# ANSSI-FR/libecc

Measured on AMD Instinct MI355X. Metric: scalar-mults/sec (secp256r1, batch=2^20, variable base, affine out, bit-exact vs CPU), higher is better.
Workload: dtype u32 (29-bit limbs, v_mad_u64_u32 integer MAD, u64 accumulators)

## Files before the change

### libecc_amd/csrc/ecamd_host.cpp

```cpp
#include <hip/hip_runtime.h>
#include <stdint.h>
#include <string.h>
#include <strings.h>
#include <stdio.h>
#include <stdlib.h>
#include <string>
#include <vector>
#include <functional>
#include <mutex>
#include <sys/random.h>

#include "../../include/libecc_amd.h"
#include "ecamd_internal.h"

static thread_local std::string g_err;
static int fail(const std::string &m)
{
	g_err = m;
	return -1;
}
#define HIPCHK(expr) \
	do { \
		hipError_t e_ = (expr); \
		if (e_ != hipSuccess) { \
// ... 1205 lines not shown
				(void)hipFree(dd);
			}
			std::vector<uint32_t> tab4((size_t)65 * 8 * 40, 0);
			for (uint32_t e = 0; ok && e < ne; e++) {
				ok = hst[e] == 0;
				big_digits29(&tab4[(size_t)e * 40], 9, big_mulmod(big_from_be(&hp[(size_t)e * 64], 32), R261, cv->p));
				big_digits29(&tab4[(size_t)e * 40 + 9], 9, big_mulmod(big_from_be(&hp[(size_t)e * 64 + 32], 32), R261, cv->p));
			}
			if (ok && hipMalloc((void **)&cv->d_comb4, tab4.size() * 4) == hipSuccess &&
			    hipMemcpy(cv->d_comb4, tab4.data(), tab4.size() * 4, hipMemcpyHostToDevice) != hipSuccess) {
				(void)hipFree(cv->d_comb4);
				cv->d_comb4 = nullptr;
			}
			(void)hipGetLastError();
		}
	}
	*out = cv;
	return 0;
}

extern "C" int ecamd_curve_by_name(ecamd_ctx *ctx, const char *name, ecamd_curve **out)
{
	if (!ctx || !name || !out) {
		return fail("ecamd_curve_by_name: NULL argument");
	}
	*out = nullptr;
	for (const CurveRow &r : g_curve_rows) {
		if (strcasecmp(r.name, name) == 0) {
			ecamd_curve *cv = new ecamd_curve();
			cv->curve_type = r.type;
			cv->p = big_from_hex(r.p);
			cv->a = big_from_hex(r.a);
			cv->b = big_from_hex(r.b);
			cv->order = big_from_hex(r.order);
			cv->gx = big_from_hex(r.gx);
			cv->gy = big_from_hex(r.gy);
			cv->q = big_from_hex(r.q);
			return curve_finish(ctx, cv, out);
		}
	}
	return fail(std::string("ecamd_curve_by_name: unknown curve ") + name);
}

extern "C" int ecamd_curve_from_params(ecamd_ctx *ctx, const uint8_t *p, uint32_t p_len, const uint8_t *a,
				       uint32_t a_len, const uint8_t *b, uint32_t b_len,
				       const uint8_t *curve_order, uint32_t curve_order_len,
				       const uint8_t *gx, uint32_t gx_len, const uint8_t *gy, uint32_t gy_len,
				       const uint8_t *gen_order, uint32_t gen_order_len, ecamd_curve **out)
{
	if (!ctx || !p || !a || !b || !curve_order || !gx || !gy || !gen_order || !out) {
		return fail("ecamd_curve_from_params: NULL argument");
	}
	*out = nullptr;
	ecamd_curve *cv = new ecamd_curve();
	cv->p = big_from_be(p, p_len);
	cv->a = big_from_be(a, a_len);
	cv->b = big_from_be(b, b_len);
	cv->order = big_from_be(curve_order, curve_order_len);
	cv->gx = big_from_be(gx, gx_len);
	cv->gy = big_from_be(gy, gy_len);
	cv->q = big_from_be(gen_order, gen_order_len);
	return curve_finish(ctx, cv, out);
}

extern "C" void ecamd_curve_free(ecamd_curve *cv)
{
	if (!cv) {
		return;
	}
	{
		std::lock_guard<std::mutex> lk(cv->ctx->mu);
		(void)hipSetDevice(cv->ctx->device);
		(void)hipStreamSynchronize(cv->ctx->stream);
		curve_free_device(cv);
	}
	curve_release_slots(cv);
	delete cv;
}

extern "C" int ecamd_curve_coord_len(const ecamd_curve *cv) { return cv ? cv->clen : -1; }
extern "C" int ecamd_curve_order_len(const ecamd_curve *cv) { return cv ? cv->qlen : -1; }
extern "C" int ecamd_curve_words(const ecamd_curve *cv) { return cv ? cv->nw : -1; }

#define P256_TAB_BYTES 512u
#define P256_SCRATCH_PER_ITEM ((size_t)P256_TAB_BYTES + 70u * 16u)

static size_t tbl_bytes_for(const ecamd_curve *cv, uint32_t stride)
{
	return (size_t)ECAMD_TBL_ENTRIES * 3 * (size_t)cv->nw * 4 * (size_t)stride;
}

static void maybe_build_comb(ecamd_ctx *ctx, ecamd_curve *cv, uint32_t n)
{
	if (cv->d_comb || cv->comb_off || ctx->comb_min_batch == 0 || n < ctx->comb_min_batch) {
		return;
	}
	const bool p256 = cv->is_p256;
	if (!p256 && cv->gslot < 0) {
		return;
	}
	cv->comb_off = true;
	if (hipDeviceSynchronize() != hipSuccess) {
		return;
	}
	const uint32_t nwords = (uint32_t)((cv->pbits + 31) / 32);
	const uint32_t slen = 4 * nwords, nwin = 2 * nwords;
	const uint32_t ne = nwin * 32768u + 1u;
	const uint32_t ew = p256 ? 20u : ecamd_g29_comb_entry_words(cv->pbits, cv->gflavour);
	if (!p256 && ne != ecamd_g29_comb_entries(cv->pbits)) {
		return;
	}
	std::vector<uint8_t> hs((size_t)ne * slen, 0);
	for (uint32_t j = 0; j < nwin; j++) {
		for (uint32_t m = 1; m <= 32768; m++) {
			uint8_t *e = &hs[((size_t)j * 32768 + (m - 1)) * slen];
			e[slen - 1 - 2 * j] = (uint8_t)(m & 0xff);
			e[slen - 2 - 2 * j] = (uint8_t)(m >> 8);
		}
	}
	big_to_be(&hs[(size_t)nwin * 32768 * slen], (int)slen, big_mod(big_pow2(8 * (int)slen), cv->q));
	const size_t plen = (size_t)2 * cv->clen;
	uint8_t *dsc = nullptr, *dpt = nullptr, *dst = nullptr;
	uint32_t *table = nullptr;
	std::vector<uint8_t> st(ne);
	hipStream_t s = ctx->stream;
	bool ok = hipMalloc((void **)&dsc, hs.size()) == hipSuccess && hipMalloc((void **)&dpt, (size_t)ne * plen) == hipSuccess &&
		  hipMalloc((void **)&dst, ne) == hipSuccess && hipMalloc((void **)&table, (size_t)ne * ew * 4) == hipSuccess &&
		  hipMemcpy(dsc, hs.data(), hs.size(), hipMemcpyHostToDevice) == hipSuccess;
	{
		const uint32_t user_chunk = ctx->max_chunk;
		ctx->max_chunk = user_chunk < (1u << 20) ? (1u << 20) : user_chunk;
		ok = ok && smul_dev_locked(ctx, cv, ne, dsc, slen, nullptr, dpt, dst, s) == 0;
		ctx->max_chunk = user_chunk;
	}
	if (ok) {
		const hipError_t e = p256 ? ecamd_launch_comb_build_p256(dpt, ne, table, s)
					  : ecamd_g29_comb_build(cv->pbits, cv->gslot, dpt, ne, (uint32_t)cv->clen, table, s, cv->gflavour);
		ok = e == hipSuccess && hipMemcpyAsync(st.data(), dst, ne, hipMemcpyDeviceToHost, s) == hipSuccess &&
		     hipStreamSynchronize(s) == hipSuccess;
	}
	for (uint32_t i = 0; ok && i < ne; i++) {
		ok = (st[i] == 0);
	}
	(void)hipFree(dsc);
	(void)hipFree(dpt);
	(void)hipFree(dst);
	if (!ok) {
		(void)hipFree(table);
		(void)hipGetLastError();
		return;
	}
	cv->d_comb = table;
	cv->comb_off = false;
}

static void maybe_build_comb4(ecamd_ctx *ctx, ecamd_curve *cv)
{
	static const bool off = getenv("ECAMD_NO_SECRET_COMB") != nullptr;
	if (off || cv->d_comb4 || cv->comb4_off || cv->is_p256 || cv->gslot < 0) {
		return;
	}
	cv->comb4_off = true;
	if (hipDeviceSynchronize() != hipSuccess) {
		return;
	}
	const uint32_t nwords = (uint32_t)((cv->pbits + 31) / 32);
	const uint32_t slen = 4 * nwords, nwin = 8 * nwords, ne = nwin * 8u + 1u;
	const uint32_t ew = ecamd_g29_comb_entry_words(cv->pbits, cv->gflavour);
// ... 4289 lines not shown
```

### libecc_amd/csrc/ecamd_internal.h

```cpp
#pragma once
#include <stdlib.h>
#include <hip/hip_runtime.h>
#include <stdint.h>

#define ECAMD_WINDOW 4
#define ECAMD_TBL_ENTRIES (1 << ECAMD_WINDOW)
#define ECAMD_STATUS_TAB 0xFC
#define ECAMD_STATUS_JAC 0xFD
#define ECAMD_STATUS_REDO 0xFE
#define ECAMD_MAX_SLOTS_HOST 16

struct EcamdSmulArgs {
	const uint8_t *scalars;
	const uint8_t *points;
	uint8_t *out;
	uint8_t *status;
	uint32_t *tbl;
	uint32_t *stg;
	uint32_t n, slen, clen, pstride, stride;
	uint32_t sstride;
	int slot;
	int only_redo;
	const uint32_t *lut;
	uint32_t lut_kind;
	int masked;
	const uint8_t *scalars2;
	uint32_t s2len;
};
#define ECAMD_COMB_ENTRIES (16u * 32768u + 1u)

struct EcamdFpArgs {
	const uint32_t *a, *b;
	uint32_t *out;
	uint32_t n, wstride;
	int op;
	int slot;
};

struct EcamdPtArgs {
	const uint8_t *p1, *p2;
	uint8_t *out, *status;
	uint32_t n, clen;
	int dbl, slot;
};

struct EcamdPtfArgs {
	const uint8_t *p1, *p2;
	uint8_t *out, *status;
	uint32_t n, clen;
	int op;
	int in_fmt, out_fmt, slot;
};
struct EcamdUnprotArgs {
	const uint8_t *points;
	const uint8_t *scalars;
	uint8_t *out, *status;
	uint32_t n, clen, slen, sstride;
	int in_fmt, out_fmt, slot;
};
hipError_t ecamd_launch_ptf(int nw, const EcamdPtfArgs &a, hipStream_t s);
hipError_t ecamd_launch_unprot(int nw, const EcamdUnprotArgs &a, hipStream_t s);

struct EcamdEcdsaPrepArgs {
	const uint8_t *sigs;
	const uint8_t *digests;
	uint8_t *u1, *u2;
	uint8_t *flags;
	uint32_t n, qlen, hlen, qbits;
	int qslot;
	const uint8_t *only;
};
struct EcamdEcdsaFinArgs {
	const uint8_t *A, *stA;
	const uint8_t *B, *stB;
	const uint8_t *sigs, *flags;
	uint8_t *result;
	uint32_t n, clen, qlen, jmax;
	uint32_t q[17];
	int slot;
	const uint8_t *only;
};
struct EcamdEcdsaSignArgs {
	const uint8_t *privs, *nonces, *digests;
	const uint8_t *kG, *stkG;
	uint8_t *sigs, *status;
	uint32_t n, clen, qlen, hlen, qbits, jmax;
	int qslot;
};
hipError_t ecamd_launch_ecdsa_sign(int nw, const EcamdEcdsaSignArgs &a, hipStream_t s);
hipError_t ecamd_launch_ecdsa_prep(int nw, const EcamdEcdsaPrepArgs &a, hipStream_t s);
hipError_t ecamd_launch_ecdsa_fin(int nw, const EcamdEcdsaFinArgs &a, hipStream_t s);

int ecamd_nw_supported(int nw);
// ... 435 lines not shown
```

### libecc_amd/csrc/ecamd_p256.h

```cpp
#pragma once
#include "ecamd_u29.h"

namespace p256 {
using namespace u29;

struct K {
	static constexpr u32 R2[9] = {0x00000c00, 0x00000000, 0x1fff0000, 0x1fdfffff, 0x1fbfffff,
				      0x1fffffff, 0x1fffffff, 0x1ffffffe, 0x00000013};
	static constexpr u32 ONE[9] = {0x00000020, 0x00000000, 0x00000000, 0x1fffc000, 0x1fffffff,
				       0x1fffffff, 0x1f7fffff, 0x03ffffff, 0x00000000};
	static constexpr u32 BM[9] = {0x1897bbfb, 0x1cdf6229, 0x018486c4, 0x01732821, 0x1dad59e0,
				      0x0abf7212, 0x1a06d110, 0x17721d20, 0x008600c3};
};

template <class T> U29_FN T constant(const u32 (&c)[9])
{
	T r;
#pragma unroll
	for (int i = 0; i < 9; i++) {
		r.l[i] = c[i];
	}
	return r;
}

// ... 57 lines not shown
	const auto t4 = sub<1, 1>(beta4, x3);
	const auto y3a = mul(alpha, t4);
	const auto y3 = carry(sub<2, 1>(y3a, g8));
	const auto z3 = mul_small<2>(mul(P.Y, P.Z));
	Jac R;
	R.X = weaken<FX>(x3);
	R.Y = weaken<FY>(y3);
	R.Z = weaken<FZ>(z3);
	return R;
}

template <class FX2, class FY2, class FZ2>
U29_FN Jac add_jac(const Jac &P, const FX2 &X2, const FY2 &Y2, const FZ2 &Z2, bool &h_is_zero)
{
	const auto z1z1 = sqr(P.Z);
	const auto z2z2 = sqr(Z2);
	const auto u1 = mul(P.X, z2z2);
	const auto u2 = mul(X2, z1z1);
	const auto s1 = mul(mul(P.Y, Z2), z2z2);
	const auto s2 = mul(mul(Y2, P.Z), z1z1);
	const auto h = carry(sub<1, 0>(u2, u1));
	const auto r = carry(sub<1, 0>(s2, s1));
	const auto hh = sqr(h);
	const auto hhh = mul(h, hh);
	const auto v = mul(u1, hh);
	const auto r2 = sqr(r);
	const auto x3 = fold(sub<2, 2>(r2, add(hhh, mul_small<2>(v))));
	const auto t5 = sub<1, 1>(v, x3);
	const auto m1 = mul(r, t5);
	const auto m2 = mul(s1, hhh);
	const auto y3 = carry(sub<1, 0>(m1, m2));
	const auto z3 = mul(mul(P.Z, Z2), h);
	h_is_zero = is_zero_mulout(z3);
	Jac R;
	R.X = weaken<FX>(x3);
	R.Y = weaken<FY>(y3);
	R.Z = weaken<FZ>(z3);
	return R;
}

typedef F<(1ull << 29) + MASK, (3ull << 24), 48> FYaff;
template <class FY2> U29_FN Jac madd(const Jac &P, const Fcanon &X2, const FY2 &Y2, bool &h_is_zero)
{
	const auto z1z1 = sqr(P.Z);
	const auto u2 = mul(X2, z1z1);
	const auto s2 = mul(mul(Y2, P.Z), z1z1);
	const auto h = carry(sub<1, 1>(u2, P.X));
	const auto r = carry(sub<3, 1>(s2, P.Y));
	const auto hh = sqr(h);
	const auto hhh = mul(h, hh);
	const auto v = mul(P.X, hh);
	const auto r2 = sqr(r);
	const auto x3 = fold(sub<2, 2>(r2, add(hhh, mul_small<2>(v))));
	const auto t5 = sub<1, 1>(v, x3);
	const auto y3 = carry(sub<1, 0>(mul(r, t5), mul(P.Y, hhh)));
	const auto z3 = mul(P.Z, h);
	h_is_zero = is_zero_mulout(z3);
	Jac R;
	R.X = weaken<FX>(x3);
	R.Y = weaken<FY>(y3);
	R.Z = weaken<FZ>(z3);
	return R;
}
U29_FN FYaff neg_aff(const Fcanon &y)
{
	F<0, 0, 0> zero;
#pragma unroll
	for (int i = 0; i < 9; i++) {
		zero.l[i] = 0;
	}
	return weaken<FYaff>(sub<1, 0>(zero, y));
}

U29_FN FYsel neg_y(const FX &y)
{
	F<0, 0, 0> zero;
#pragma unroll
	for (int i = 0; i < 9; i++) {
		zero.l[i] = 0;
	}
	return weaken<FYsel>(carry(sub<1, 1>(zero, y)));
}

U29_FN TabEnt to_tab(const Jac &P)
{
	TabEnt T;
	T.X = P.X;
	T.Y = weaken<FX>(fold(P.Y));
	T.Z = P.Z;
	return T;
}

}
```

### libecc_amd/csrc/ecamd_p256_kernel.hip

```cpp
#include <hip/hip_runtime.h>
#include "ecamd_p256.h"
#include "ecamd_internal.h"

using namespace p256;

typedef uint8_t u8;

#define TBL_WORDS_PER_ENTRY 40
#define TBL_ENTRIES 8
#define TAB_ENT_WORDS 16
#define TAB_ITEM_WORDS (TBL_ENTRIES * TAB_ENT_WORDS)
#define STG_ENT_QUADS 10
#define STG_ITEM_QUADS (7 * STG_ENT_QUADS)
#ifndef FIN_K
#define FIN_K 8
#endif
#ifndef AFF_K
#define AFF_K 8
#endif
static inline int p256_items_per_inversion(uint32_t n, int kmax)
{
	const int k = n >= (1u << 19) ? 8 : (n >= (1u << 17) ? 4 : 2);
	return k < kmax ? k : kmax;
}

static __device__ __forceinline__ void load_be256(const u8 *src, u32 *w)
{
	if ((((uintptr_t)src) & 15) == 0) {
		const uint4 a = *(const uint4 *)src, b = *(const uint4 *)(src + 16);
		w[7] = __builtin_bswap32(a.x);
		w[6] = __builtin_bswap32(a.y);
		w[5] = __builtin_bswap32(a.z);
		w[4] = __builtin_bswap32(a.w);
		w[3] = __builtin_bswap32(b.x);
		w[2] = __builtin_bswap32(b.y);
		w[1] = __builtin_bswap32(b.z);
		w[0] = __builtin_bswap32(b.w);
	} else {
#pragma unroll
		for (int i = 0; i < 8; i++) {
			const u8 *q = src + 4 * (7 - i);
			w[i] = ((u32)q[0] << 24) | ((u32)q[1] << 16) | ((u32)q[2] << 8) | (u32)q[3];
		}
	}
}

static __device__ __forceinline__ void store_be256(u8 *dst, const u32 *w)
{
	if ((((uintptr_t)dst) & 15) == 0) {
		uint4 a, b;
		a.x = __builtin_bswap32(w[7]);
		a.y = __builtin_bswap32(w[6]);
		a.z = __builtin_bswap32(w[5]);
		a.w = __builtin_bswap32(w[4]);
		b.x = __builtin_bswap32(w[3]);
		b.y = __builtin_bswap32(w[2]);
		b.z = __builtin_bswap32(w[1]);
		b.w = __builtin_bswap32(w[0]);
		*(uint4 *)dst = a;
		*(uint4 *)(dst + 16) = b;
	} else {
#pragma unroll
		for (int i = 0; i < 8; i++) {
			u8 *q = dst + 4 * (7 - i);
			q[0] = (u8)(w[i] >> 24);
			q[1] = (u8)(w[i] >> 16);
			q[2] = (u8)(w[i] >> 8);
			q[3] = (u8)w[i];
		}
	}
}

static __device__ __forceinline__ bool lt_p(const u32 *w)
{
	constexpr u32 pw[8] = {0xffffffffu, 0xffffffffu, 0xffffffffu, 0x00000000u, 0x00000000u, 0x00000000u, 0x00000001u, 0xffffffffu};
	u32 borrow = 0;
#pragma unroll
	for (int i = 0; i < 8; i++) {
		const uint64_t x = (uint64_t)w[i] - pw[i] - borrow;
		borrow = (u32)(x >> 63);
	}
	return borrow != 0;
}

static __device__ __forceinline__ uint4 *stg_quad(u32 *stg, u32 i, int slot, int q)
{
	return (uint4 *)stg + ((size_t)(i >> 6) * STG_ITEM_QUADS + (size_t)(slot * STG_ENT_QUADS + q)) * 64 + (i & 63u);
}
static __device__ __forceinline__ void jac_store(u32 *stg, u32 i, int slot, const Jac &P)
{
	u32 b[28];
#pragma unroll
	for (int w = 0; w < 9; w++) {
		b[w] = P.X.l[w];
		b[9 + w] = P.Y.l[w];
		b[18 + w] = P.Z.l[w];
	}
	b[27] = 0;
#pragma unroll
	for (int q = 0; q < 7; q++) {
		*stg_quad(stg, i, slot, q) = make_uint4(b[4 * q], b[4 * q + 1], b[4 * q + 2], b[4 * q + 3]);
	}
}
static __device__ __forceinline__ Jac jac_load(u32 *stg, u32 i, int slot)
{
	u32 b[28];
#pragma unroll
	for (int q = 0; q < 7; q++) {
		const uint4 v = *stg_quad(stg, i, slot, q);
		b[4 * q] = v.x; b[4 * q + 1] = v.y; b[4 * q + 2] = v.z; b[4 * q + 3] = v.w;
	}
	Jac P;
#pragma unroll
	for (int w = 0; w < 9; w++) {
		P.X.l[w] = b[w];
		P.Y.l[w] = b[9 + w];
		P.Z.l[w] = b[18 + w];
	}
	return P;
}
static __device__ __forceinline__ FZ z_load(u32 *stg, u32 i, int slot)
{
	u32 b[12];
#pragma unroll
	for (int q = 0; q < 3; q++) {
		const uint4 v = *stg_quad(stg, i, slot, 4 + q);
		b[4 * q] = v.x; b[4 * q + 1] = v.y; b[4 * q + 2] = v.z; b[4 * q + 3] = v.w;
	}
	FZ z;
#pragma unroll
	for (int w = 0; w < 9; w++) {
		z.l[w] = b[2 + w];
	}
	return z;
}
static __device__ __forceinline__ void prefix_store(u32 *stg, u32 i, int slot, const Fmul &c)
{
	*stg_quad(stg, i, slot, 7) = make_uint4(c.l[0], c.l[1], c.l[2], c.l[3]);
	*stg_quad(stg, i, slot, 8) = make_uint4(c.l[4], c.l[5], c.l[6], c.l[7]);
	*stg_quad(stg, i, slot, 9) = make_uint4(c.l[8], 0u, 0u, 0u);
}
static __device__ __forceinline__ Fmul prefix_load(u32 *stg, u32 i, int slot)
{
	const uint4 a = *stg_quad(stg, i, slot, 7), b = *stg_quad(stg, i, slot, 8), c = *stg_quad(stg, i, slot, 9);
	Fmul r;
	r.l[0] = a.x; r.l[1] = a.y; r.l[2] = a.z; r.l[3] = a.w;
	r.l[4] = b.x; r.l[5] = b.y; r.l[6] = b.z; r.l[7] = b.w;
	r.l[8] = c.x;
	return r;
}

static __device__ __forceinline__ void tab_store(u32 *tab, u32 i, int e, const Fcanon &x, const Fcanon &y)
{
	u32 w[16];
	to_words(w, x);
	to_words(w + 8, y);
	uint4 *d = (uint4 *)(tab + (size_t)i * TAB_ITEM_WORDS + e * TAB_ENT_WORDS);
#pragma unroll
	for (int q = 0; q < 4; q++) {
		d[q] = make_uint4(w[4 * q], w[4 * q + 1], w[4 * q + 2], w[4 * q + 3]);
	}
}
static __device__ __forceinline__ void tab_load(const u32 *tab, u32 e, Fcanon &x, Fcanon &y)
{
	u32 w[16];
	const uint4 *s = (const uint4 *)(tab + (size_t)e * TAB_ENT_WORDS);
#pragma unroll
	for (int q = 0; q < 4; q++) {
		const uint4 v = s[q];
		w[4 * q] = v.x; w[4 * q + 1] = v.y; w[4 * q + 2] = v.z; w[4 * q + 3] = v.w;
	}
	x = from_words(w);
	y = from_words(w + 8);
}
static __device__ __forceinline__ void tab_load_masked(const u32 *tab, u32 idx, Fcanon &x, Fcanon &y)
{
	u32 w[16];
#pragma unroll
	for (int k = 0; k < 16; k++) {
		w[k] = 0;
	}
#pragma unroll 1
	for (u32 e = 0; e < TBL_ENTRIES; e++) {
		const uint4 *s = (const uint4 *)(tab + (size_t)e * TAB_ENT_WORDS);
		const u32 m = 0u - (u32)(e == idx);
#pragma unroll
		for (int q = 0; q < 4; q++) {
			const uint4 v = s[q];
			w[4 * q] |= v.x & m; w[4 * q + 1] |= v.y & m; w[4 * q + 2] |= v.z & m; w[4 * q + 3] |= v.w & m;
		}
	}
	x = from_words(w);
	y = from_words(w + 8);
}
template <int NQ> static __device__ __forceinline__ void ld(u32 *b, const u32 *s)
{
	const uint4 *q = (const uint4 *)s;
#pragma unroll
	for (int i = 0; i < NQ; i++) {
		const uint4 v = q[i];
		b[4 * i] = v.x;
		b[4 * i + 1] = v.y;
		b[4 * i + 2] = v.z;
		b[4 * i + 3] = v.w;
	}
}
static __device__ __forceinline__ void lut_load_masked(const u32 *lut, u32 idx, Fcanon &x, Fcanon &y);
static __device__ __forceinline__ void lut_load(const u32 *lut, size_t e, Fcanon &x, Fcanon &y)
{
	u32 b[20];
	ld<5>(b, lut + e * TBL_WORDS_PER_ENTRY);
#pragma unroll
	for (int w = 0; w < 9; w++) {
		x.l[w] = b[w];
		y.l[w] = b[9 + w];
	}
}

template <class T> static __device__ __forceinline__ T sel(bool c, const T &a, const T &b)
{
	T r;
#pragma unroll
	for (int i = 0; i < 9; i++) {
		r.l[i] = c ? a.l[i] : b.l[i];
	}
	return r;
}

static __device__ __forceinline__ void zero_out(u8 *out)
{
	const uint4 z = make_uint4(0, 0, 0, 0);
	if ((((uintptr_t)out) & 15) == 0) {
		((uint4 *)out)[0] = z; ((uint4 *)out)[1] = z; ((uint4 *)out)[2] = z; ((uint4 *)out)[3] = z;
	} else {
		for (int b = 0; b < 64; b++) out[b] = 0;
	}
}

__global__ __launch_bounds__(64) void k_p256_table(EcamdSmulArgs A)
{
	const u32 i = blockIdx.x * 64 + threadIdx.x;
	if (i >= A.n) {
		return;
	}
	const u8 *pin = A.points + (size_t)i * A.pstride;
	u32 xw[8], yw[8];
	load_be256(pin, xw);
	load_be256(pin + 32, yw);
	bool ok = lt_p(xw) & lt_p(yw);
	const Fcanon r2 = constant<Fcanon>(K::R2);
	const auto xm = mul(from_words(xw), r2);
	const auto ym = mul(from_words(yw), r2);
	{
		const auto x3 = mul(sqr(xm), xm);
		const auto rhs = sub<3, 2>(add(x3, constant<Fcanon>(K::BM)), mul_small<3>(xm));
		const auto dif = carry(sub<1, 0>(carry(rhs), sqr(ym)));
		ok = ok & is_zero_mulout(mul(dif, constant<Fcanon>(K::ONE)));
	}
	if (!ok) {
		A.status[i] = 1;
		zero_out(A.out + (size_t)i * 64);
		return;
	}
	const Fcanon xa = canonical(xm), ya = canonical(ym);
	tab_store(A.tbl, i, 0, xa, ya);
	Jac P1;
	P1.X = weaken<FX>(xm);
	P1.Y = weaken<FY>(ym);
	P1.Z = weaken<FZ>(constant<Fcanon>(K::ONE));
	bool hz;
	const FYaff y1 = weaken<FYaff>(ya);
	Jac Pa = dbl(P1);
	jac_store(A.stg, i, 0, Pa);
	Jac Pb = madd(Pa, xa, y1, hz);
	jac_store(A.stg, i, 1, Pb);
	Pa = dbl(Pa);
	jac_store(A.stg, i, 2, Pa);
	Pb = madd(Pa, xa, y1, hz);
	jac_store(A.stg, i, 3, Pb);
	Pb = dbl(jac_load(A.stg, i, 1));
	jac_store(A.stg, i, 4, Pb);
	Pb = madd(Pb, xa, y1, hz);
	jac_store(A.stg, i, 5, Pb);
	Pa = dbl(Pa);
	jac_store(A.stg, i, 6, Pa);
	A.status[i] = ECAMD_STATUS_TAB;
}

__global__ __launch_bounds__(64) void k_p256_affine(EcamdSmulArgs A, u32 nthreads, int items)
{
	const u32 t = blockIdx.x * 64 + threadIdx.x;
	if (t >= nthreads) {
		return;
	}
	Fmul c = weaken<Fmul>(constant<Fcanon>(K::ONE));
#pragma unroll 1
	for (int j = 0; j < items; j++) {
		const u32 i = t + (u32)j * nthreads;
		if (i >= A.n) {
			break;
		}
		if (A.status[i] != ECAMD_STATUS_TAB) {
			continue;
		}
#pragma unroll 1
		for (int e = 0; e < 7; e++) {
			const FZ z = z_load(A.stg, i, e);
			prefix_store(A.stg, i, e, c);
			c = weaken<Fmul>(mul(c, z));
		}
	}
	Fmul tinv = inv(c);
#pragma unroll 1
	for (int j = items - 1; j >= 0; j--) {
		const u32 i = t + (u32)j * nthreads;
		if (i >= A.n || A.status[i] != ECAMD_STATUS_TAB) {
			continue;
		}
#pragma unroll 1
		for (int e = 6; e >= 0; e--) {
			const Jac P = jac_load(A.stg, i, e);
			const Fmul cbf = prefix_load(A.stg, i, e);
			const Fmul zi = weaken<Fmul>(mul(tinv, cbf));
			tinv = weaken<Fmul>(mul(tinv, P.Z));
			const Fmul zi2 = weaken<Fmul>(sqr(zi));
			const Fmul zi3 = weaken<Fmul>(mul(zi2, zi));
			const Fcanon ax = canonical(mul(P.X, zi2));
			const Fcanon ay = canonical(mul(P.Y, zi3));
			tab_store(A.tbl, i, e + 1, ax, ay);
		}
	}
}

#ifndef P256_WAVES
#define P256_WAVES 3
#endif
template <int KW> static __device__ __forceinline__ u32 recode_window(u32 *kw, const u8 *sc, int slen)
{
	if (KW == 8 && slen == 32) {
		load_be256(sc, kw);
	} else {
#pragma unroll
		for (int w = 0; w < KW; w++) {
			u32 x = 0;
// ... 58 lines not shown
		x.l[w] = b[w];
		y.l[w] = b[9 + w];
	}
}

template <int KW, bool MASKED>
__global__ __launch_bounds__(64) __attribute__((amdgpu_waves_per_eu(P256_WAVES, P256_WAVES))) void k_p256_loop(EcamdSmulArgs A)
{
	const u32 i = blockIdx.x * 64 + threadIdx.x;
	if (i >= A.n || A.status[i] != ECAMD_STATUS_TAB) {
		return;
	}
	const u32 *tabi = A.tbl + (size_t)i * TAB_ITEM_WORDS;
	const bool shared = A.lut != nullptr;
	const int slen = (int)A.slen;
	u32 kw[KW];
	const u32 carry_bit = recode_window<KW>(kw, A.scalars + (size_t)i * A.sstride, slen);

	Jac acc;
	{
		Fcanon px, py;
		if (shared) {
			lut_load(A.lut, 0, px, py);
		} else {
			tab_load(tabi, 0, px, py);
		}
		acc.X = weaken<FX>(px);
		acc.Y = weaken<FY>(py);
		acc.Z = weaken<FZ>(constant<Fcanon>(K::ONE));
	}
	bool inf = (carry_bit == 0);
	bool bad = false, hz;
	const int nwin = 2 * slen;
	const FZ onez = weaken<FZ>(constant<Fcanon>(K::ONE));
#pragma unroll 1
	for (int t = 0; t < nwin; t++) {
#pragma unroll 1
		for (int d = 0; d < 4; d++) {
			acc = dbl(acc);
		}
		const int dig = (int)(kw[KW - 1] >> 28) - 8;
#pragma unroll
		for (int w = KW - 1; w > 0; w--) {
			kw[w] = (kw[w] << 4) | (kw[w - 1] >> 28);
		}
		kw[0] <<= 4;
		const u32 mag = (u32)(dig < 0 ? -dig : dig);
		Fcanon tx, tyc;
		const u32 idx = mag ? mag - 1 : 0;
		if (MASKED) {
			if (shared) {
				lut_load_masked(A.lut, idx, tx, tyc);
			} else {
				tab_load_masked(tabi, idx, tx, tyc);
			}
		} else if (shared) {
			lut_load(A.lut, idx, tx, tyc);
		} else {
			tab_load(tabi, idx, tx, tyc);
		}
		const FYaff ty = sel(dig < 0, neg_aff(tyc), weaken<FYaff>(tyc));
		const Jac S = madd(acc, tx, ty, hz);
		const bool use_t = inf & (mag != 0);
		const bool keep = (mag == 0);
		bad = bad | (!inf & !keep & hz);
		acc.X = sel(keep, acc.X, sel(use_t, weaken<FX>(tx), S.X));
		acc.Y = sel(keep, acc.Y, sel(use_t, weaken<FY>(carry(ty)), S.Y));
		acc.Z = sel(keep, acc.Z, sel(use_t, onez, S.Z));
		inf = inf & keep;
	}
	if (bad) {
		A.status[i] = ECAMD_STATUS_REDO;
		return;
	}
	if (inf) {
		A.status[i] = 2;
		zero_out(A.out + (size_t)i * 64);
		return;
	}
	jac_store(A.stg, i, 0, acc);
	A.status[i] = ECAMD_STATUS_JAC;
}

#define COMB_ENT_WORDS 20
#define COMB_PER_WIN 32768

__global__ __launch_bounds__(64) void k_p256_comb_build(const u8 *pts, u32 n, u32 *table)
{
	const u32 i = blockIdx.x * 64 + threadIdx.x;
	if (i >= n) {
		return;
	}
	u32 xw[8], yw[8];
	load_be256(pts + (size_t)i * 64, xw);
	load_be256(pts + (size_t)i * 64 + 32, yw);
	const Fcanon r2 = constant<Fcanon>(K::R2);
	const Fcanon xa = canonical(mul(from_words(xw), r2)), ya = canonical(mul(from_words(yw), r2));
	u32 b[20];
#pragma unroll
	for (int w = 0; w < 9; w++) {
		b[w] = xa.l[w];
		b[9 + w] = ya.l[w];
	}
	b[18] = b[19] = 0;
	uint4 *d = (uint4 *)(table + (size_t)i * COMB_ENT_WORDS);
#pragma unroll
	for (int q = 0; q < 5; q++) {
		d[q] = make_uint4(b[4 * q], b[4 * q + 1], b[4 * q + 2], b[4 * q + 3]);
	}
}

static __device__ __forceinline__ u32 comb_recode(u32 *kw, const u8 *sc, int slen)
{
	if (slen == 32) {
		load_be256(sc, kw);
	} else {
#pragma unroll
		for (int w = 0; w < 8; w++) {
			u32 x = 0;
#pragma unroll
			for (int b = 0; b < 4; b++) {
				const int pos = 4 * w + b;
				if (pos < slen) {
					x |= (u32)sc[slen - 1 - pos] << (8 * b);
				}
			}
			kw[w] = x;
		}
	}
	uint64_t c = 0;
#pragma unroll
	for (int w = 0; w < 8; w++) {
		c += (uint64_t)kw[w] + 0x80008000u;
		kw[w] = (u32)c;
		c >>= 32;
	}
	return (u32)c;
}

static __device__ __forceinline__ void comb_accumulate(Jac &acc, bool &inf, bool &bad, const u32 *kw, u32 top, const u32 *comb)
{
	const FZ onez = weaken<FZ>(constant<Fcanon>(K::ONE));
#pragma unroll 1
	for (int j = 0; j <= 16; j++) {
		const int dig = (j < 16) ? (int)((kw[j >> 1] >> (16 * (j & 1))) & 0xffffu) - 0x8000 : (int)top;
		const u32 mag = (u32)(dig < 0 ? -dig : dig);
		u32 b[20];
		ld<5>(b, comb + ((size_t)j * COMB_PER_WIN + (mag ? mag - 1 : 0)) * COMB_ENT_WORDS);
		Fcanon tx, tyc;
#pragma unroll
		for (int w = 0; w < 9; w++) {
			tx.l[w] = b[w];
			tyc.l[w] = b[9 + w];
		}
		const FYaff ty = sel(dig < 0, neg_aff(tyc), weaken<FYaff>(tyc));
		bool hz;
		const Jac S = madd(acc, tx, ty, hz);
		const bool use_t = inf & (mag != 0);
		const bool keep = (mag == 0);
		bad = bad | (!inf & !keep & hz);
		acc.X = sel(keep, acc.X, sel(use_t, weaken<FX>(tx), S.X));
		acc.Y = sel(keep, acc.Y, sel(use_t, weaken<FY>(carry(ty)), S.Y));
		acc.Z = sel(keep, acc.Z, sel(use_t, onez, S.Z));
		inf = inf & keep;
	}
}
// ... 268 lines not shown
		u32 cy = 0;
#pragma unroll
		for (int w = 0; w < 9; w++) {
			const u32 x = rd.l[w] + A.qd[w] + cy;
			cy = (w < 8) ? (x >> 29) : 0u;
			sdg[w] = (w < 8) ? (x & MASK) : x;
		}
		u32 bw = 0;
#pragma unroll
		for (int w = 0; w < 9; w++) {
			bw = (sdg[w] - P256::P[w] - bw) >> 31;
		}
		Fcanon rq;
#pragma unroll
		for (int w = 0; w < 9; w++) {
			rq.l[w] = bw ? sdg[w] : 0u;
		}
		const auto t2 = mul(mul(rq, r2c), z2);
		acc_ok = acc_ok | ((bw != 0) & is_zero_mulout(mul(carry(sub<1, 1>(t2, acc.X)), onec)));
	}
	A.result[i] = acc_ok ? 0 : 1;
}

hipError_t ecamd_launch_verify_p256(const EcamdSmulArgs &pubkeys, const uint8_t *u1, const uint8_t *u2, const uint8_t *sigs,
				    const uint8_t *flags, const uint32_t *gtbl, int gtbl_is_comb, const uint32_t *qdigits,
				    uint8_t *result, hipStream_t s, hipEvent_t *dom, hipEvent_t scalars_ready)
{
	if (pubkeys.n == 0) {
		return scalars_ready ? hipStreamWaitEvent(s, scalars_ready, 0) : hipSuccess;
	}
	const dim3 grid((pubkeys.n + 63) / 64), block(64);
	const uint32_t ak = (uint32_t)p256_items_per_inversion(pubkeys.n, AFF_K);
	const uint32_t athreads = (((pubkeys.n + ak - 1) / ak) + 63u) & ~63u;
	hipLaunchKernelGGL(k_p256_table, grid, block, 0, s, pubkeys);
	hipLaunchKernelGGL(k_p256_affine, dim3((athreads + 63) / 64), block, 0, s, pubkeys, athreads, (int)ak);
	P256VerifyArgs V;
	V.u1 = u1;
	V.u2 = u2;
	V.sigs = sigs;
	V.flags = flags;
	V.status = pubkeys.status;
	V.qtbl = pubkeys.tbl;
	V.gtbl = gtbl;
	V.result = result;
	V.n = pubkeys.n;
	for (int w = 0; w < 9; w++) {
		V.qd[w] = qdigits[w];
	}
	if (scalars_ready) {
		const hipError_t e = hipStreamWaitEvent(s, scalars_ready, 0);
		if (e != hipSuccess) {
			return e;
		}
	}
	if (dom) {
		(void)hipEventRecord(dom[0], s);
	}
	if (gtbl_is_comb) {
		hipLaunchKernelGGL(k_p256_verify_loop<true>, grid, block, 0, s, V);
	} else {
		hipLaunchKernelGGL(k_p256_verify_loop<false>, grid, block, 0, s, V);
	}
	if (dom) {
		(void)hipEventRecord(dom[1], s);
	}
	return hipGetLastError();
}

hipError_t ecamd_launch_smul_p256(const EcamdSmulArgs &a, hipStream_t s, hipEvent_t *ev)
{
	if (a.n == 0) {
		return hipSuccess;
	}
	const dim3 grid((a.n + 63) / 64), block(64);
	const uint32_t fk = (uint32_t)p256_items_per_inversion(a.n, FIN_K);
	const uint32_t nthreads = (((a.n + fk - 1) / fk) + 63u) & ~63u;
	const dim3 fgrid((nthreads + 63) / 64);
#define P256_MARK(i) do { if (ev) (void)hipEventRecord(ev[i], s); } while (0)
	P256_MARK(0);
	if (a.lut) {
		(void)hipMemsetAsync(a.status, ECAMD_STATUS_TAB, a.n, s);
		P256_MARK(1);
	} else {
		hipLaunchKernelGGL(k_p256_table, grid, block, 0, s, a);
		P256_MARK(1);
		const uint32_t ak = (uint32_t)p256_items_per_inversion(a.n, AFF_K);
		const uint32_t athreads = (((a.n + ak - 1) / ak) + 63u) & ~63u;
		hipLaunchKernelGGL(k_p256_affine, dim3((athreads + 63) / 64), block, 0, s, a, athreads, (int)ak);
	}
	P256_MARK(2);
	if (a.lut && a.lut_kind == 1) {
		hipLaunchKernelGGL(k_p256_comb, grid, block, 0, s, a);
	} else if (a.lut && a.lut_kind == 3) {
		hipLaunchKernelGGL(k_p256_comb4m, grid, block, 0, s, a);
	} else {
		if (a.masked) {
			if (a.slen <= 32) {
				hipLaunchKernelGGL((k_p256_loop<8, true>), grid, block, 0, s, a);
			} else {
				hipLaunchKernelGGL((k_p256_loop<17, true>), grid, block, 0, s, a);
			}
		} else if (a.slen <= 32) {
			hipLaunchKernelGGL((k_p256_loop<8, false>), grid, block, 0, s, a);
		} else {
			hipLaunchKernelGGL((k_p256_loop<17, false>), grid, block, 0, s, a);
		}
	}
	P256_MARK(3);
	hipLaunchKernelGGL(k_p256_finalize, fgrid, block, 0, s, a, nthreads, (int)fk);
	P256_MARK(4);
	return hipGetLastError();
}

hipError_t ecamd_launch_comb_build_p256(const uint8_t *points, uint32_t n, uint32_t *table, hipStream_t s)
{
	if (n == 0) {
		return hipSuccess;
	}
	hipLaunchKernelGGL(k_p256_comb_build, dim3((n + 63) / 64), dim3(64), 0, s, points, n, table);
	return hipGetLastError();
}
```

Baseline: 74.43 million.

## Use odd-digit signed windows with co-Z precomputation for P-256 variable-base path

Replaces the 8-entry window table with an odd-multiples table {1,3,...,15}P. The table is built via co-Z DBLU/ZADDU steps, and the z ratios are stored so a single batched inversion can convert all entries to affine. The scalar is recoded, made odd by adding the group order when it is even, into signed odd 4-bit digits. This removes the special-casing of zero digits and makes every window a fixed dbl^4 plus mixed add. It cuts table-building cost (co-Z adds are cheaper than full Jacobian adds) and gives a constant add per window, at the price of new recoding logic and a different scratch layout.

Result: faster. 76.12 million, median of 6 (+2.3%).

```diff
diff --git a/libecc_amd/csrc/ecamd_host.cpp b/libecc_amd/csrc/ecamd_host.cpp
--- a/libecc_amd/csrc/ecamd_host.cpp
+++ b/libecc_amd/csrc/ecamd_host.cpp
@@ -1311,8 +1311,7 @@
 extern "C" int ecamd_curve_order_len(const ecamd_curve *cv) { return cv ? cv->qlen : -1; }
 extern "C" int ecamd_curve_words(const ecamd_curve *cv) { return cv ? cv->nw : -1; }
 
-#define P256_TAB_BYTES 512u
-#define P256_SCRATCH_PER_ITEM ((size_t)P256_TAB_BYTES + 70u * 16u)
+#define P256_SCRATCH_PER_ITEM ((size_t)P256_TAB_BYTES + P256_STG_QUADS * 16u)
 
 static size_t tbl_bytes_for(const ecamd_curve *cv, uint32_t stride)
 {
diff --git a/libecc_amd/csrc/ecamd_internal.h b/libecc_amd/csrc/ecamd_internal.h
--- a/libecc_amd/csrc/ecamd_internal.h
+++ b/libecc_amd/csrc/ecamd_internal.h
@@ -9,6 +9,8 @@
 #define ECAMD_STATUS_JAC 0xFD
 #define ECAMD_STATUS_REDO 0xFE
 #define ECAMD_MAX_SLOTS_HOST 16
+#define P256_TAB_BYTES 512u
+#define P256_STG_QUADS 70u
 
 struct EcamdSmulArgs {
 	const uint8_t *scalars;
diff --git a/libecc_amd/csrc/ecamd_p256.h b/libecc_amd/csrc/ecamd_p256.h
--- a/libecc_amd/csrc/ecamd_p256.h
+++ b/libecc_amd/csrc/ecamd_p256.h
@@ -163,6 +163,100 @@
 	return weaken<FYsel>(carry(sub<1, 1>(zero, y)));
 }
 
+typedef F<MASK + 16, (2ull << 24), 32> FXc;
+typedef F<MASK + 16, (4ull << 24), 63> FYc;
+typedef F<MASK + 15, (8ull << 24), 128> FR;
+struct CoZ {
+	FXc X;
+	FYc Y;
+};
+
+template <class AX, class AY> U29_FN void dblu(const AX &x, const AY &y, CoZ &D, CoZ &P1, FZ &z)
+{
+	const Fcanon one = constant<Fcanon>(K::ONE);
+	const auto gamma = sqr(y);
+	const auto beta4 = mul(x, mul_small<4>(gamma));
+	const auto t1 = sub<1, 0>(x, one);
+	const auto t2 = add(x, one);
+	const auto alpha = carry(mul_small<3>(mul(t1, t2)));
+	const auto a2 = sqr(alpha);
+	const auto x3 = fold(sub<2, 1>(a2, mul_small<2>(beta4)));
+	const auto g8 = mul_small<2>(sqr(mul_small<2>(gamma)));
+	const auto y3 = fold(sub<2, 2>(mul(alpha, sub<1, 1>(beta4, x3)), g8));
+	D.X = weaken<FXc>(x3);
+	D.Y = weaken<FYc>(y3);
+	P1.X = weaken<FXc>(beta4);
+	P1.Y = weaken<FYc>(carry(g8));
+	z = weaken<FZ>(mul_small<2>(y));
+}
+
+U29_FN void zaddu(CoZ &P1, const CoZ &P2, CoZ &R, FR &r)
+{
+	const auto h = carry(sub<2, 1>(P1.X, P2.X));
+	const auto c = sqr(h);
+	const auto w1 = mul(P1.X, c);
+	const auto w2 = mul(P2.X, c);
+	const auto dy = carry(sub<2, 1>(P1.Y, P2.Y));
+	const auto d = sqr(dy);
+	const auto a1 = mul(P1.Y, sub<1, 0>(w1, w2));
+	const auto x3 = fold(sub<2, 1>(d, add(w1, w2)));
+	const auto y3 = carry(sub<1, 0>(mul(dy, sub<1, 1>(w1, x3)), a1));
+	R.X = weaken<FXc>(x3);
+	R.Y = weaken<FYc>(y3);
+	P1.X = weaken<FXc>(w1);
+	P1.Y = weaken<FYc>(a1);
+	r = weaken<FR>(h);
+}
+
+struct QOrder {
+	static constexpr u32 W[8] = {0xfc632551u, 0xf3b9cac2u, 0xa7179e84u, 0xbce6faadu, 0xffffffffu, 0xffffffffu, 0x00000000u, 0xffffffffu};
+};
+template <int KW, int WB> U29_FN int recode_odd(u32 *e, const u32 *kw, int slen)
+{
+	constexpr int NW = KW + 1;
+	const u32 even = (kw[0] & 1u) - 1u;
+	u64 c = 0;
+#pragma unroll
+	for (int w = 0; w < KW; w++) {
+		c += (u64)kw[w] + (w < 8 ? (QOrder::W[w] & even) : 0u);
+		e[w] = (u32)c;
+		c >>= 32;
+	}
+	e[KW] = (u32)c;
+	e[0] &= ~1u;
+	const int nbits = (KW == 8) ? 257 : ((8 * slen > 256 ? 8 * slen : 256) + 1);
+	const int t = (nbits + WB - 1) / WB;
+	const int sh = 32 * NW - WB * t - 1;
+	for (int s = 0; s < (sh >> 5); s++) {
+#pragma unroll
+		for (int w = NW - 1; w > 0; w--) {
+			e[w] = e[w - 1];
+		}
+		e[0] = 0;
+	}
+	const int bs = sh & 31;
+#pragma unroll
+	for (int w = NW - 1; w > 0; w--) {
+		e[w] = (u32)((((u64)e[w] << 32) | e[w - 1]) >> (32 - bs));
+	}
+	e[0] = (u32)(((u64)e[0] << 32) >> (32 - bs));
+	e[NW - 1] |= 0x80000000u;
+	return t;
+}
+template <int NW, int WB> U29_FN bool odd_digit(u32 *e, u32 &idx)
+{
+	constexpr u32 HALF = 1u << (WB - 1);
+	const u32 win = e[NW - 1] >> (32 - WB);
+#pragma unroll
+	for (int w = NW - 1; w > 0; w--) {
+		e[w] = (e[w] << WB) | (e[w - 1] >> (32 - WB));
+	}
+	e[0] <<= WB;
+	const bool neg = win < HALF;
+	idx = (win & (HALF - 1)) ^ (neg ? HALF - 1 : 0u);
+	return neg;
+}
+
 U29_FN TabEnt to_tab(const Jac &P)
 {
 	TabEnt T;
diff --git a/libecc_amd/csrc/ecamd_p256_kernel.hip b/libecc_amd/csrc/ecamd_p256_kernel.hip
--- a/libecc_amd/csrc/ecamd_p256_kernel.hip
+++ b/libecc_amd/csrc/ecamd_p256_kernel.hip
@@ -12,6 +12,7 @@
 #define TAB_ITEM_WORDS (TBL_ENTRIES * TAB_ENT_WORDS)
 #define STG_ENT_QUADS 10
 #define STG_ITEM_QUADS (7 * STG_ENT_QUADS)
+static_assert(TAB_ITEM_WORDS * 4 <= P256_TAB_BYTES && STG_ITEM_QUADS <= P256_STG_QUADS, "scratch exceeds the host's per-item sizing");
 #ifndef FIN_K
 #define FIN_K 8
 #endif
@@ -150,12 +151,13 @@
 	return r;
 }
 
+template <int ITEM_WORDS = TAB_ITEM_WORDS>
 static __device__ __forceinline__ void tab_store(u32 *tab, u32 i, int e, const Fcanon &x, const Fcanon &y)
 {
 	u32 w[16];
 	to_words(w, x);
 	to_words(w + 8, y);
-	uint4 *d = (uint4 *)(tab + (size_t)i * TAB_ITEM_WORDS + e * TAB_ENT_WORDS);
+	uint4 *d = (uint4 *)(tab + (size_t)i * ITEM_WORDS + e * TAB_ENT_WORDS);
 #pragma unroll
 	for (int q = 0; q < 4; q++) {
 		d[q] = make_uint4(w[4 * q], w[4 * q + 1], w[4 * q + 2], w[4 * q + 3]);
@@ -173,6 +175,7 @@
 	x = from_words(w);
 	y = from_words(w + 8);
 }
+template <u32 NENT = TBL_ENTRIES>
 static __device__ __forceinline__ void tab_load_masked(const u32 *tab, u32 idx, Fcanon &x, Fcanon &y)
 {
 	u32 w[16];
@@ -181,7 +184,7 @@
 		w[k] = 0;
 	}
 #pragma unroll 1
-	for (u32 e = 0; e < TBL_ENTRIES; e++) {
+	for (u32 e = 0; e < NENT; e++) {
 		const uint4 *s = (const uint4 *)(tab + (size_t)e * TAB_ENT_WORDS);
 		const u32 m = 0u - (u32)(e == idx);
 #pragma unroll
@@ -237,20 +240,17 @@
 	}
 }
 
-__global__ __launch_bounds__(64) void k_p256_table(EcamdSmulArgs A)
-{
-	const u32 i = blockIdx.x * 64 + threadIdx.x;
-	if (i >= A.n) {
-		return;
-	}
+typedef MulOut<17>::type PtIn;
+static __device__ __forceinline__ bool import_point(const EcamdSmulArgs &A, u32 i, PtIn &xm, PtIn &ym)
+{
 	const u8 *pin = A.points + (size_t)i * A.pstride;
 	u32 xw[8], yw[8];
 	load_be256(pin, xw);
 	load_be256(pin + 32, yw);
 	bool ok = lt_p(xw) & lt_p(yw);
 	const Fcanon r2 = constant<Fcanon>(K::R2);
-	const auto xm = mul(from_words(xw), r2);
-	const auto ym = mul(from_words(yw), r2);
+	xm = mul(from_words(xw), r2);
+	ym = mul(from_words(yw), r2);
 	{
 		const auto x3 = mul(sqr(xm), xm);
 		const auto rhs = sub<3, 2>(add(x3, constant<Fcanon>(K::BM)), mul_small<3>(xm));
@@ -260,6 +260,18 @@
 	if (!ok) {
 		A.status[i] = 1;
 		zero_out(A.out + (size_t)i * 64);
+	}
+	return ok;
+}
+
+__global__ __launch_bounds__(64) void k_p256_table(EcamdSmulArgs A)
+{
+	const u32 i = blockIdx.x * 64 + threadIdx.x;
+	if (i >= A.n) {
+		return;
+	}
+	PtIn xm, ym;
+	if (!import_point(A, i, xm, ym)) {
 		return;
 	}
 	const Fcanon xa = canonical(xm), ya = canonical(ym);
@@ -484,6 +496,211 @@
 	A.status[i] = ECAMD_STATUS_JAC;
 }
 
+#ifndef P256_ODD_WINDOWS
+#define P256_ODD_WINDOWS 1
+#endif
+#define ODD_WB 4
+#define ODD_NE (1 << (ODD_WB - 1))
+#define ODD_TAB_ITEM_WORDS (ODD_NE * TAB_ENT_WORDS)
+#define ODD_ENT_QUADS 7
+#define ODD_ZQ ((ODD_NE - 1) * ODD_ENT_QUADS)
+#define ODD_ITEM_QUADS (ODD_ZQ + 6)
+static_assert(ODD_TAB_ITEM_WORDS * 4 <= P256_TAB_BYTES && ODD_ITEM_QUADS <= P256_STG_QUADS, "odd-window scratch exceeds the host's per-item sizing");
+
+static __device__ __forceinline__ uint4 *odd_quad(u32 *stg, u32 i, int q)
+{
+	return (uint4 *)stg + ((size_t)(i >> 6) * ODD_ITEM_QUADS + (size_t)q) * 64 + (i & 63u);
+}
+template <class T> static __device__ __forceinline__ void odd_store9(u32 *stg, u32 i, int q, const T &a)
+{
+	*odd_quad(stg, i, q) = make_uint4(a.l[0], a.l[1], a.l[2], a.l[3]);
+	*odd_quad(stg, i, q + 1) = make_uint4(a.l[4], a.l[5], a.l[6], a.l[7]);
+	*odd_quad(stg, i, q + 2) = make_uint4(a.l[8], 0u, 0u, 0u);
+}
+template <class T> static __device__ __forceinline__ T odd_load9(u32 *stg, u32 i, int q)
+{
+	const uint4 a = *odd_quad(stg, i, q), b = *odd_quad(stg, i, q + 1), c = *odd_quad(stg, i, q + 2);
+	T r;
+	r.l[0] = a.x; r.l[1] = a.y; r.l[2] = a.z; r.l[3] = a.w;
+	r.l[4] = b.x; r.l[5] = b.y; r.l[6] = b.z; r.l[7] = b.w;
+	r.l[8] = c.x;
+	return r;
+}
+static __device__ __forceinline__ void odd_ent_store(u32 *stg, u32 i, int e, const CoZ &T, const FR &r)
+{
+	u32 b[28];
+#pragma unroll
+	for (int w = 0; w < 9; w++) {
+		b[w] = T.X.l[w];
+		b[9 + w] = T.Y.l[w];
+		b[18 + w] = r.l[w];
+	}
+	b[27] = 0;
+#pragma unroll
+	for (int q = 0; q < ODD_ENT_QUADS; q++) {
+		*odd_quad(stg, i, (e - 1) * ODD_ENT_QUADS + q) = make_uint4(b[4 * q], b[4 * q + 1], b[4 * q + 2], b[4 * q + 3]);
+	}
+}
+static __device__ __forceinline__ void odd_ent_load(u32 *stg, u32 i, int e, CoZ &T, FR &r)
+{
+	u32 b[28];
+#pragma unroll
+	for (int q = 0; q < ODD_ENT_QUADS; q++) {
+		const uint4 v = *odd_quad(stg, i, (e - 1) * ODD_ENT_QUADS + q);
+		b[4 * q] = v.x; b[4 * q + 1] = v.y; b[4 * q + 2] = v.z; b[4 * q + 3] = v.w;
+	}
+#pragma unroll
+	for (int w = 0; w < 9; w++) {
+		T.X.l[w] = b[w];
+		T.Y.l[w] = b[9 + w];
+		r.l[w] = b[18 + w];
+	}
+}
+
+__global__ __launch_bounds__(64) void k_p256_table_odd(EcamdSmulArgs A)
+{
+	const u32 i = blockIdx.x * 64 + threadIdx.x;
+	if (i >= A.n) {
+		return;
+	}
+	PtIn xm, ym;
+	if (!import_point(A, i, xm, ym)) {
+		return;
+	}
+	tab_store<ODD_TAB_ITEM_WORDS>(A.tbl, i, 0, canonical(xm), canonical(ym));
+	CoZ D, T;
+	FZ z;
+	dblu(xm, ym, D, T, z);
+#pragma unroll 1
+	for (int e = 1; e < ODD_NE; e++) {
+		CoZ Tn;
+		FR r;
+		zaddu(D, T, Tn, r);
+		z = weaken<FZ>(mul(z, r));
+		odd_ent_store(A.stg, i, e, Tn, r);
+		T = Tn;
+	}
+	odd_store9(A.stg, i, ODD_ZQ, z);
+	A.status[i] = ECAMD_STATUS_TAB;
+}
+
+__global__ __launch_bounds__(64) void k_p256_affine_coz(EcamdSmulArgs A, u32 nthreads, int items)
+{
+	const u32 t = blockIdx.x * 64 + threadIdx.x;
+	if (t >= nthreads) {
+		return;
+	}
+	Fmul c = weaken<Fmul>(constant<Fcanon>(K::ONE));
+#pragma unroll 1
+	for (int j = 0; j < items; j++) {
+		const u32 i = t + (u32)j * nthreads;
+		if (i >= A.n) {
+			break;
+		}
+		if (A.status[i] != ECAMD_STATUS_TAB) {
+			continue;
+		}
+		const FZ z = odd_load9<FZ>(A.stg, i, ODD_ZQ);
+		odd_store9(A.stg, i, ODD_ZQ + 3, c);
+		c = weaken<Fmul>(mul(c, z));
+	}
+	Fmul tinv = inv(c);
+#pragma unroll 1
+	for (int j = items - 1; j >= 0; j--) {
+		const u32 i = t + (u32)j * nthreads;
+		if (i >= A.n || A.status[i] != ECAMD_STATUS_TAB) {
+			continue;
+		}
+		Fmul zi = weaken<Fmul>(mul(tinv, odd_load9<Fmul>(A.stg, i, ODD_ZQ + 3)));
+		tinv = weaken<Fmul>(mul(tinv, odd_load9<FZ>(A.stg, i, ODD_ZQ)));
+#pragma unroll 1
+		for (int e = ODD_NE - 1; e >= 1; e--) {
+			CoZ T;
+			FR r;
+			odd_ent_load(A.stg, i, e, T, r);
+			const Fmul zi2 = weaken<Fmul>(sqr(zi));
+			const Fmul zi3 = weaken<Fmul>(mul(zi2, zi));
+			tab_store<ODD_TAB_ITEM_WORDS>(A.tbl, i, e, canonical(mul(T.X, zi2)), canonical(mul(T.Y, zi3)));
+			if (e > 1) {
+				zi = weaken<Fmul>(mul(zi, r));
+			}
+		}
+	}
+}
+
+template <int KW, bool MASKED>
+__global__ __launch_bounds__(64) __attribute__((amdgpu_waves_per_eu(P256_WAVES, P256_WAVES))) void k_p256_loop_odd(EcamdSmulArgs A)
+{
+	const u32 i = blockIdx.x * 64 + threadIdx.x;
+	if (i >= A.n || A.status[i] != ECAMD_STATUS_TAB) {
+		return;
+	}
+	const u32 *tabi = A.tbl + (size_t)i * ODD_TAB_ITEM_WORDS;
+	const int slen = (int)A.slen;
+	u32 e[KW + 1];
+	int nwin;
+	{
+		u32 kw[KW];
+		const u8 *sc = A.scalars + (size_t)i * A.sstride;
+		if (KW == 8 && slen == 32) {
+			load_be256(sc, kw);
+		} else {
+#pragma unroll
+			for (int w = 0; w < KW; w++) {
+				u32 x = 0;
+#pragma unroll
+				for (int b = 0; b < 4; b++) {
+					const int pos = 4 * w + b;
+					if (pos < slen) {
+						x |= (u32)sc[slen - 1 - pos] << (8 * b);
+					}
+				}
+				kw[w] = x;
+			}
+		}
+		nwin = recode_odd<KW, ODD_WB>(e, kw, slen);
+	}
+	Jac acc;
+	{
+		u32 idx;
+		(void)odd_digit<KW + 1, ODD_WB>(e, idx);
+		Fcanon px, py;
+		if (MASKED) {
+			tab_load_masked<ODD_NE>(tabi, idx, px, py);
+		} else {
+			tab_load(tabi, idx, px, py);
+		}
+		acc.X = weaken<FX>(px);
+		acc.Y = weaken<FY>(py);
+		acc.Z = weaken<FZ>(constant<Fcanon>(K::ONE));
+	}
+	bool bad = false, hz;
+#pragma unroll 1
+	for (int t = 1; t < nwin; t++) {
+#pragma unroll 1
+		for (int d = 0; d < ODD_WB; d++) {
+			acc = dbl(acc);
+		}
+		u32 idx;
+		const bool neg = odd_digit<KW + 1, ODD_WB>(e, idx);
+		Fcanon tx, tyc;
+		if (MASKED) {
+			tab_load_masked<ODD_NE>(tabi, idx, tx, tyc);
+		} else {
+			tab_load(tabi, idx, tx, tyc);
+		}
+		const FYaff ty = sel(neg, neg_aff(tyc), weaken<FYaff>(tyc));
+		acc = madd(acc, tx, ty, hz);
+		bad = bad | hz;
+	}
+	if (bad) {
+		A.status[i] = ECAMD_STATUS_REDO;
+		return;
+	}
+	jac_store(A.stg, i, 0, acc);
+	A.status[i] = ECAMD_STATUS_JAC;
+}
+
 #define COMB_ENT_WORDS 20
 #define COMB_PER_WIN 32768
 
@@ -918,14 +1135,32 @@
 		(void)hipMemsetAsync(a.status, ECAMD_STATUS_TAB, a.n, s);
 		P256_MARK(1);
 	} else {
-		hipLaunchKernelGGL(k_p256_table, grid, block, 0, s, a);
-		P256_MARK(1);
 		const uint32_t ak = (uint32_t)p256_items_per_inversion(a.n, AFF_K);
 		const uint32_t athreads = (((a.n + ak - 1) / ak) + 63u) & ~63u;
-		hipLaunchKernelGGL(k_p256_affine, dim3((athreads + 63) / 64), block, 0, s, a, athreads, (int)ak);
+		if (P256_ODD_WINDOWS) {
+			hipLaunchKernelGGL(k_p256_table_odd, grid, block, 0, s, a);
+			P256_MARK(1);
+			hipLaunchKernelGGL(k_p256_affine_coz, dim3((athreads + 63) / 64), block, 0, s, a, athreads, (int)ak);
+		} else {
+			hipLaunchKernelGGL(k_p256_table, grid, block, 0, s, a);
+			P256_MARK(1);
+			hipLaunchKernelGGL(k_p256_affine, dim3((athreads + 63) / 64), block, 0, s, a, athreads, (int)ak);
+		}
 	}
 	P256_MARK(2);
-	if (a.lut && a.lut_kind == 1) {
+	if (!a.lut && P256_ODD_WINDOWS) {
+		if (a.masked) {
+			if (a.slen <= 32) {
+				hipLaunchKernelGGL((k_p256_loop_odd<8, true>), grid, block, 0, s, a);
+			} else {
+				hipLaunchKernelGGL((k_p256_loop_odd<17, true>), grid, block, 0, s, a);
+			}
+		} else if (a.slen <= 32) {
+			hipLaunchKernelGGL((k_p256_loop_odd<8, false>), grid, block, 0, s, a);
+		} else {
+			hipLaunchKernelGGL((k_p256_loop_odd<17, false>), grid, block, 0, s, a);
+		}
+	} else if (a.lut && a.lut_kind == 1) {
 		hipLaunchKernelGGL(k_p256_comb, grid, block, 0, s, a);
 	} else if (a.lut && a.lut_kind == 3) {
 		hipLaunchKernelGGL(k_p256_comb4m, grid, block, 0, s, a);
```
